# MengRao/pollnet

Measured on AMD Instinct MI355X. Metric: device-resident Gbit/s + Mframes/s, 1500 B IPv4/TCP frames, 1/2/4/8 MI355X, higher is better.
Workload: dtype u16/u32 integer (one's-complement sums)

## Files before the change

include/pollnet_amd.h:

```cpp
#ifndef POLLNET_AMD_H
#define POLLNET_AMD_H

#include <stdint.h>

#ifdef __cplusplus
extern "C" {
#endif

#define PN_ABI_VERSION 1

#define PN_RECV_BUF_SIZE 2048u
#define PN_RECV_MSS 1460u
#define PN_EMPTY_KEY (1ull << 63)
#define PN_MISS 0xFFFFFFFFu

#define PN_OK 0
#define PN_EINVAL -1
#define PN_EHIP -2
#define PN_ENOMEM -3
#define PN_ENOTABLE -4
#define PN_EFULL -5
#define PN_ENOENT -6

typedef struct pn_result {
  uint32_t conn_id;
  uint32_t seq;
  uint16_t payload_off;
  int16_t payload_len;
  uint16_t flags;
  uint16_t tcp_fold;
} pn_result;

#define PN_F_IP_OK 0x0001u
#define PN_F_TCP_OK 0x0002u
#define PN_F_HIT 0x0004u
#define PN_F_TW 0x0008u
#define PN_F_FIN 0x0010u
#define PN_F_SYN 0x0020u
#define PN_F_RST 0x0040u
#define PN_F_PSH 0x0080u
#define PN_F_ACK 0x0100u
#define PN_F_IHL_NE_5 0x0200u
#define PN_F_RFC_IP_OK 0x0400u
#define PN_F_RFC_TCP_OK 0x0800u
#define PN_F_NOT_TCP 0x1000u
#define PN_F_TRUNC 0x2000u
#define PN_F_BADOFF 0x4000u
#define PN_F_TCP_UNCHECKED 0x8000u

typedef struct pn_conn_entry {
  uint64_t key;
  uint32_t conn_id;
  uint32_t _pad;
} pn_conn_entry;

typedef struct pn_conn_table pn_conn_table;

uint64_t pn_conn_hash_key(uint32_t ip_be, uint16_t port_be);

int pn_table_create(uint32_t max_conn_cnt, uint32_t max_tw_cnt, pn_conn_table** out);
#define PN_TABLE_REFERENCE_LITERAL 1u
int pn_table_create_ex(uint32_t max_conn_cnt, uint32_t max_tw_cnt, uint32_t flags, pn_conn_table** out);
uint32_t pn_table_flags(const pn_conn_table* t);
void pn_table_destroy(pn_conn_table* t);
int pn_table_find(const pn_conn_table* t, uint64_t key, uint32_t* entry_idx, int* hit, uint32_t* conn_id);
int pn_table_add(pn_conn_table* t, uint64_t key, uint32_t conn_id);
int pn_table_del(pn_conn_table* t, uint64_t key);
int pn_table_set_conn_id(pn_conn_table* t, uint64_t key, uint32_t conn_id);
const pn_conn_entry* pn_table_entries(const pn_conn_table* t, uint32_t* n_entries, uint64_t* tbl_mask);
uint32_t pn_table_max_conn_cnt(const pn_conn_table* t);
uint32_t pn_table_size(const pn_conn_table* t);
uint32_t pn_table_repairs(const pn_conn_table* t);

typedef struct pn_ctx pn_ctx;

int pn_open(int device, pn_ctx** out);
void pn_close(pn_ctx* ctx);
const char* pn_last_error(const pn_ctx* ctx);
int pn_device_count(int* n);

int pn_set_conn_table(pn_ctx* ctx, const pn_conn_entry* entries, uint32_t n_entries, uint64_t tbl_mask,
                      uint32_t max_conn_cnt);

int pn_set_verify(pn_ctx* ctx, int verify_tcp);

int pn_classify(pn_ctx* ctx, const void* frames_dev, uint32_t slot_stride, uint32_t frame_off, uint32_t n,
                void* results_dev, void* stream);

int pn_classify_indexed(pn_ctx* ctx, const void* base, const uint64_t* offsets, uint32_t eth_mod16, uint32_t n,
                        uint32_t avail, void* results, void* stream);

#define PN_MAX_STREAM_FILTERS 64
#define PN_NO_STREAM 0xFFFFFFFFu
typedef struct pn_stream_filter {
  uint32_t src_ip;
  uint32_t dst_ip;
  uint16_t src_port;
  uint16_t dst_port;
  uint32_t _pad;
} pn_stream_filter;

int pn_match_streams(pn_ctx* ctx, const void* frames, uint32_t slot_stride, uint32_t frame_off, uint32_t n,
                     const pn_stream_filter* filters, uint32_t n_filters, uint32_t* stream_ids, void* stream);

#define PN_UDP_MAX_SUBS 4096u
#define PN_UDP_NO_SUB 0xFFFFFFFFu
typedef struct pn_udp_sub {
  uint32_t dst_ip;
  uint16_t dst_port;
  uint16_t _pad;
} pn_udp_sub;

typedef struct pn_udp_result {
  uint32_t sub_id;
  uint32_t src_ip;
  uint16_t src_port;
  uint16_t payload_off;
  uint16_t payload_len;
  uint16_t flags;
} pn_udp_result;

#define PN_UF_IP_OK 0x0001u
#define PN_UF_UDP_OK 0x0002u
#define PN_UF_MATCH 0x0004u
#define PN_UF_NOCSUM 0x0008u
#define PN_UF_FRAG 0x0010u
#define PN_UF_LEN_BAD 0x0020u
#define PN_UF_IHL_NE_5 0x0200u
#define PN_UF_NOT_UDP 0x1000u
#define PN_UF_TRUNC 0x2000u
#define PN_UF_BADOFF 0x4000u
#define PN_UF_UDP_UNCHECKED 0x8000u
#define PN_UDP_DELIVER(f) (((f) & PN_UF_MATCH) && ((f) & PN_UF_IP_OK) && \
                           ((f) & (PN_UF_UDP_OK | PN_UF_NOCSUM | PN_UF_UDP_UNCHECKED)))

int pn_udp_set_subs(pn_ctx* ctx, const pn_udp_sub* subs, uint32_t n_subs);
int pn_udp_classify(pn_ctx* ctx, const void* frames, uint32_t slot_stride, uint32_t frame_off, uint32_t n,
                    void* results, void* stream);
int pn_udp_classify_indexed(pn_ctx* ctx, const void* base, const uint64_t* offsets, uint32_t eth_mod16,
                            uint32_t n, uint32_t avail, void* results, void* stream);

#define PN_UDP_MAX_CHANNELS 4096u
typedef struct pn_udp_channel {
  uint8_t hdr[42];
  uint8_t _pad[6];
} pn_udp_channel;

#define PN_UB_EFVI 0u
#define PN_UB_PLAIN 1u
#define PN_UB_CSUM 2u

int pn_udp_set_channels(pn_ctx* ctx, const pn_udp_channel* chans, uint32_t n_chans);
int pn_udp_build(pn_ctx* ctx, const void* payloads, uint64_t payload_bytes, const uint64_t* pay_offs,
                 const uint16_t* pay_lens, const uint32_t* chan_ids, void* frames, uint32_t slot_stride,
                 uint32_t frame_off, uint32_t n, uint32_t mode, uint16_t* frame_lens, void* stream);

#define PN_UDP_GATHER_ALIGN 16u
typedef struct pn_udp_gather_total {
  uint64_t n_bytes;
  uint32_t n_msgs;
  uint32_t n_fit;
} pn_udp_gather_total;

int pn_udp_gather(pn_ctx* ctx, const void* frames, uint32_t slot_stride, uint32_t frame_off, uint32_t n,
                  const void* results, void* payloads, uint64_t payload_cap, uint64_t* pay_offs, uint16_t* pay_lens,
                  uint32_t* sub_ids, uint32_t* src_index, pn_udp_gather_total* total, void* stream);
int pn_udp_gather_indexed(pn_ctx* ctx, const void* base, const uint64_t* offsets, uint32_t eth_mod16, uint32_t n,
                          uint32_t avail, const void* results, void* payloads, uint64_t payload_cap,
                          uint64_t* pay_offs, uint16_t* pay_lens, uint32_t* sub_ids, uint32_t* src_index,
                          pn_udp_gather_total* total, void* stream);

#define PN_TX_TCP 0u
#define PN_TX_UDP_EFVI 1u
#define PN_TX_UDP 2u
int pn_tx_fill(pn_ctx* ctx, void* frames, uint32_t slot_stride, uint32_t frame_off, uint32_t n, const uint16_t* lens,
               uint32_t mode, void* stream);

#define PN_NOTIFY_MAX_FRAMES 1024u
int pn_classify_notify(pn_ctx* ctx, const void* frames, uint32_t slot_stride, uint32_t frame_off, uint32_t n,
                       void* results, void* stream, uint32_t* done_word, uint32_t token);
int pn_tx_fill_notify(pn_ctx* ctx, void* frames, uint32_t slot_stride, uint32_t frame_off, uint32_t n,
                      const uint16_t* lens, uint32_t mode, void* stream, uint32_t* done_word, uint32_t token);

typedef struct pn_service pn_service;
#define PN_SERVICE_WAVES 64u
#define PN_SERVICE_WAVES_PER_CU 12u
#define PN_SERVICE_MAX_WAVES 4096u
#define PN_SERVICE_MAX_FRAMES (1u << 20)
#define PN_SERVICE_STOP 0xFFFFFFFFu
int pn_service_open(pn_ctx* ctx, uint32_t slot_stride, uint32_t frame_off, uint32_t idle_ms, pn_service** out);
int pn_service_open_ex(pn_ctx* ctx, uint32_t slot_stride, uint32_t frame_off, uint32_t idle_ms, uint32_t large_waves,
                       pn_service** out);
int pn_service_post(pn_service* svc, const void* frames, uint32_t n, void* results, uint32_t* post_id);
#define PN_LINK_MAX_FRAMES 1024u
#define PN_LINK_MAX_CONNS 4096u
int pn_service_post_linked(pn_service* svc, const void* frames, uint32_t n, void* results, uint16_t* links,
                           uint32_t* post_id);
int pn_service_wait(pn_service* svc, uint32_t post_id);
int pn_service_close(pn_service* svc);

int pn_sync(pn_ctx* ctx);

#ifdef __cplusplus
}
#endif
#endif
```

pollnet_amd/__init__.py:

```python
from .rx import (
    LIB_PATH,
    PN_EMPTY_KEY,
    PN_MISS,
    PN_TX_TCP,
    PN_TX_UDP_EFVI,
    PN_TX_UDP,
    RESULT_DTYPE,
    ENTRY_DTYPE,
    STREAM_FILTER_DTYPE,
    PN_NO_STREAM,
    PN_MAX_STREAM_FILTERS,
    UDP_SUB_DTYPE,
    UDP_RESULT_DTYPE,
    PN_UDP_NO_SUB,
    PN_UDP_MAX_SUBS,
    UDP_CHANNEL_DTYPE,
    PN_UDP_MAX_CHANNELS,
    UDP_GATHER_TOTAL_DTYPE,
    PN_UDP_GATHER_ALIGN,
    PN_UB_EFVI,
    PN_UB_PLAIN,
    PN_UB_CSUM,
    UF,
    PN_SERVICE_WAVES,
    PN_SERVICE_WAVES_PER_CU,
    PN_SERVICE_MAX_WAVES,
    PN_SERVICE_MAX_FRAMES,
    PN_LINK_MAX_FRAMES,
    PN_LINK_MAX_CONNS,
    F,
    ConnTable,
    PollnetError,
    RxContext,
    RxService,
    conn_hash_key,
    device_count,
    gen_conn_table,
    gen_frames,
    wire_bytes,
)
```

pollnet_amd/csrc/conn_table.cpp:

```cpp
#include <algorithm>
#include <cstdint>
#include <cstring>
#include <new>
#include <utility>
#include <vector>

#include "../../include/pollnet_amd.h"

namespace {

constexpr int msb_count(uint32_t n) { return n == 0 ? 0 : msb_count(n >> 1) + 1; }

struct ConnTable {
  std::vector<pn_conn_entry> tbl;
  uint64_t mask = 0;
  uint32_t max_conn = 0, max_tw = 0, size = 0;
  uint32_t repairs = 0;
  bool literal = false;

  bool init(uint32_t mc, uint32_t mtw, bool lit) {
    literal = lit;
    max_conn = mc;
    max_tw = mtw;
    uint64_t max_tbl = 1ull << (1 + msb_count(mc + mtw));
    if (max_tbl > (1ull << 28)) return false;
    tbl.assign(max_tbl + mc + mtw, pn_conn_entry{PN_EMPTY_KEY, 0, 0});
    mask = std::min<uint64_t>(max_tbl, 128) - 1;
    size = 0;
    return true;
  }

  uint32_t find(uint64_t key) const {
    uint64_t e = key & mask;
    const uint64_t n = tbl.size();
    while (e < n && tbl[e].key < key) ++e;
    return (uint32_t)e;
  }

  void insert_sorted(uint64_t key, uint32_t conn_id) {
    uint32_t e = find(key);
    while (tbl[e].key != PN_EMPTY_KEY) {
      std::swap(tbl[e].key, key);
      std::swap(tbl[e].conn_id, conn_id);
      while (tbl[++e].key < key) {
      }
    }
    tbl[e].key = key;
    tbl[e].conn_id = conn_id;
  }

  void expand() {
    if ((uint64_t)size * 2 <= mask) return;
    std::vector<pn_conn_entry> saved;
    saved.reserve(size);
    for (const auto& x : tbl)
      if (x.key != PN_EMPTY_KEY) saved.push_back(x);
    bool broken = false;
    uint64_t end = mask + 1;
    mask = mask * 2 + 1;
    uint64_t new_end = mask + 1;
    while (tbl[end].key != PN_EMPTY_KEY) std::swap(tbl[new_end++], tbl[end++]);
    const uint64_t end_cnt = new_end - (mask + 1);
    auto rehash = [&](uint64_t e, uint64_t cnt) {
      for (; cnt; ++e) {
        if (tbl[e].key == PN_EMPTY_KEY) continue;
        uint32_t ne = find(tbl[e].key);
        if (tbl[ne].key != tbl[e].key && tbl[ne].key != PN_EMPTY_KEY) broken = true;
        std::swap(tbl[e].key, tbl[ne].key);
        tbl[ne].conn_id = tbl[e].conn_id;
        --cnt;
      }
    };
    rehash(0, size - end_cnt);
    rehash(mask + 1, end_cnt);
    if (broken && !literal) {
      ++repairs;
      for (auto& x : tbl) x = pn_conn_entry{PN_EMPTY_KEY, 0, 0};
      for (const auto& x : saved) insert_sorted(x.key, x.conn_id);
    }
  }

  int add(uint64_t key, uint32_t conn_id) {
    uint32_t e = find(key);
    if (e < tbl.size() && tbl[e].key == key) return PN_EINVAL;
    if (size >= max_conn + max_tw) return PN_EFULL;
    ++size;
    insert_sorted(key, conn_id);
    expand();
    return PN_OK;
  }

  int del(uint64_t key) {
    uint32_t e = find(key);
    if (e >= tbl.size() || tbl[e].key != key) return PN_ENOENT;
    --size;
    for (;;) {
      uint32_t next = e + 1;
      while ((tbl[next].key & mask) > e) ++next;
      if (tbl[next].key == PN_EMPTY_KEY) break;
      tbl[e] = tbl[next];
      e = next;
    }
    tbl[e].key = PN_EMPTY_KEY;
    return PN_OK;
  }
};

}

struct pn_conn_table {
  ConnTable t;
};

extern "C" {

uint64_t pn_conn_hash_key(uint32_t ip_be, uint16_t port_be) {
  uint64_t ip = __builtin_bswap32(ip_be);
  uint64_t p = __builtin_bswap16(port_be);
  return (ip << 15) | (p & 0x7fff) | ((p & 0x8000) << 32);
}

int pn_table_create(uint32_t max_conn_cnt, uint32_t max_tw_cnt, pn_conn_table** out) {
  return pn_table_create_ex(max_conn_cnt, max_tw_cnt, 0, out);
}

int pn_table_create_ex(uint32_t max_conn_cnt, uint32_t max_tw_cnt, uint32_t flags, pn_conn_table** out) {
  if (!out || max_conn_cnt == 0 || (flags & ~PN_TABLE_REFERENCE_LITERAL)) return PN_EINVAL;
  auto* t = new (std::nothrow) pn_conn_table();
  if (!t) return PN_ENOMEM;
  if (!t->t.init(max_conn_cnt, max_tw_cnt, flags & PN_TABLE_REFERENCE_LITERAL)) {
    delete t;
    return PN_EINVAL;
  }
  *out = t;
  return PN_OK;
}

void pn_table_destroy(pn_conn_table* t) { delete t; }

int pn_table_find(const pn_conn_table* t, uint64_t key, uint32_t* entry_idx, int* hit, uint32_t* conn_id) {
  if (!t) return PN_EINVAL;
  uint32_t e = t->t.find(key);
  bool h = e < t->t.tbl.size() && t->t.tbl[e].key == key;
  if (entry_idx) *entry_idx = e;
  if (hit) *hit = h;
  if (conn_id) *conn_id = h ? t->t.tbl[e].conn_id : PN_MISS;
  return PN_OK;
}

int pn_table_add(pn_conn_table* t, uint64_t key, uint32_t conn_id) {
  if (!t || key >= PN_EMPTY_KEY) return PN_EINVAL;
  return t->t.add(key, conn_id);
}

int pn_table_del(pn_conn_table* t, uint64_t key) {
  if (!t) return PN_EINVAL;
  return t->t.del(key);
}

int pn_table_set_conn_id(pn_conn_table* t, uint64_t key, uint32_t conn_id) {
  if (!t) return PN_EINVAL;
  uint32_t e = t->t.find(key);
  if (e >= t->t.tbl.size() || t->t.tbl[e].key != key) return PN_ENOENT;
  t->t.tbl[e].conn_id = conn_id;
  return PN_OK;
}

const pn_conn_entry* pn_table_entries(const pn_conn_table* t, uint32_t* n_entries, uint64_t* tbl_mask) {
  if (!t) return nullptr;
  if (n_entries) *n_entries = (uint32_t)t->t.tbl.size();
  if (tbl_mask) *tbl_mask = t->t.mask;
  return t->t.tbl.data();
}

uint32_t pn_table_max_conn_cnt(const pn_conn_table* t) { return t ? t->t.max_conn : 0; }
uint32_t pn_table_size(const pn_conn_table* t) { return t ? t->t.size : 0; }
uint32_t pn_table_repairs(const pn_conn_table* t) { return t ? t->t.repairs : 0; }
uint32_t pn_table_flags(const pn_conn_table* t) { return t && t->t.literal ? PN_TABLE_REFERENCE_LITERAL : 0u; }

}
```

pollnet_amd/csrc/pn_internal.hpp:

```cpp
#pragma once

#include <hip/hip_runtime.h>

#include <cstdint>
#include <string>
#include <vector>

#include "../../include/pollnet_amd.h"

struct pn_fence {
  hipStream_t s = nullptr;
  hipEvent_t ev = nullptr;
  uint8_t state = 0;
};

struct pn_ctx {
  int device = 0;
  pn_conn_entry* tbl_buf[2] = {nullptr, nullptr};
  uint32_t tbl_cap[2] = {0, 0};
  int cur = 0;
  pn_conn_entry* tbl_dev = nullptr;
  uint32_t n_entries = 0;
  uint64_t mask = 0;
  uint32_t max_conn = 0;
  bool verify_tcp = true;
  std::vector<hipStream_t> streams;
  std::vector<hipEvent_t> retired;
  size_t n_retired = 0;
  hipStream_t copy_stream = nullptr;
  void* tx_patch = nullptr;
  uint32_t tx_patch_n = 0;
  pn_fence tx;
  void* sig_count = nullptr;
  pn_fence sig[2];
  std::vector<pn_service*> services;
  uint64_t* udp_tbl = nullptr;
  uint32_t udp_cap = 0;
  uint32_t udp_mask = 0;
  uint32_t udp_n = 0;
  uint32_t* ub_tbl = nullptr;
  uint32_t ub_cap = 0;
  uint32_t ub_n = 0;
  void* ug_scratch = nullptr;
  uint32_t ug_scratch_n = 0;
  pn_fence ug;
  std::string err;
};

namespace pn_internal {

inline thread_local std::string g_err;

inline int set_err(pn_ctx* ctx, int code, const std::string& msg) {
  if (ctx) ctx->err = msg;
  g_err = msg;
  return code;
}

int svc_release_table(pn_ctx* ctx, int buf);

inline int hip_err(pn_ctx* ctx, hipError_t e, const char* what) {
  return set_err(ctx, PN_EHIP, std::string(what) + ": " + hipGetErrorString(e));
}

inline void note_stream(pn_ctx* ctx, hipStream_t s) {
  if (!ctx->streams.empty() && ctx->streams.back() == s) return;
  for (size_t i = 0; i < ctx->streams.size(); ++i)
    if (ctx->streams[i] == s) {
      std::swap(ctx->streams[i], ctx->streams.back());
      return;
    }
  ctx->streams.push_back(s);
}

inline int ensure_event(pn_ctx* ctx, hipEvent_t* ev) {
  if (*ev) return PN_OK;
  hipError_t e = hipEventCreateWithFlags(ev, hipEventDisableTiming);
  if (e != hipSuccess) return hip_err(ctx, e, "hipEventCreate");
  return PN_OK;
}

inline int fence_host_wait(pn_ctx* ctx, pn_fence& f) {
  hipError_t e = hipSuccess;
  if (f.state == 1) e = hipStreamSynchronize(f.s);
  else if (f.state == 2) e = hipEventSynchronize(f.ev);
  if (e != hipSuccess) return hip_err(ctx, e, "waiting for the last user of ctx scratch");
  f.state = 0;
  return PN_OK;
}

inline int fence_use(pn_ctx* ctx, pn_fence& f, hipStream_t s) {
  hipError_t e = hipSuccess;
  if (f.state == 1 && f.s != s) {
    int rc = ensure_event(ctx, &f.ev);
    if (rc) return rc;
    e = hipEventRecord(f.ev, f.s);
    if (e == hipSuccess) e = hipStreamWaitEvent(s, f.ev, 0);
  } else if (f.state == 2) {
    e = hipStreamWaitEvent(s, f.ev, 0);
  }
  if (e != hipSuccess) return hip_err(ctx, e, "ordering after the previous user of ctx scratch");
  f.s = s;
  f.state = 1;
  return PN_OK;
}

inline int fence_detach(pn_ctx* ctx, pn_fence& f) {
  if (f.state != 1) return PN_OK;
  int rc = ensure_event(ctx, &f.ev);
  if (rc) return rc;
  hipError_t e = hipEventRecord(f.ev, f.s);
  if (e != hipSuccess) return hip_err(ctx, e, "hipEventRecord(ctx scratch fence)");
  f.state = 2;
  f.s = nullptr;
  return PN_OK;
}

inline int wait_retired(pn_ctx* ctx) {
  for (size_t i = 0; i < ctx->n_retired; ++i) {
    hipError_t e = hipEventSynchronize(ctx->retired[i]);
    if (e != hipSuccess) return hip_err(ctx, e, "hipEventSynchronize(previous table readers)");
  }
  ctx->n_retired = 0;
  return PN_OK;
}

inline int retire_streams(pn_ctx* ctx) {
  for (size_t i = 0; i < ctx->streams.size(); ++i) {
    if (ctx->retired.size() <= i) ctx->retired.push_back(nullptr);
    int rc = ensure_event(ctx, &ctx->retired[i]);
    if (rc) return rc;
    hipError_t e = hipEventRecord(ctx->retired[i], ctx->streams[i]);
    if (e != hipSuccess) return hip_err(ctx, e, "hipEventRecord(table readers)");
  }
  ctx->n_retired = ctx->streams.size();
  ctx->streams.clear();
  for (pn_fence* f : {&ctx->sig[0], &ctx->sig[1], &ctx->tx, &ctx->ug}) {
    int rc = fence_detach(ctx, *f);
    if (rc) return rc;
  }
  return PN_OK;
}

inline int notify_counter(pn_ctx* ctx, int kind, hipStream_t s, uint32_t** out) {
  hipError_t e;
  if (!ctx->sig_count) {
    e = hipMalloc(&ctx->sig_count, 128);
    if (e == hipSuccess) e = hipMemsetAsync(ctx->sig_count, 0, 128, s);
    if (e != hipSuccess) return hip_err(ctx, e, "hipMalloc(notify counters)");
    for (pn_fence& f : ctx->sig) {
      f.s = s;
      f.state = 1;
    }
    note_stream(ctx, s);
  }
  int rc = fence_use(ctx, ctx->sig[kind], s);
  if (rc) return rc;
  *out = (uint32_t*)ctx->sig_count + 16 * kind;
  return PN_OK;
}

}
```

pollnet_amd/csrc/rx_kernel.hip:

```cpp
#include "rx_classify.hpp"

namespace {
using pn_internal::g_err;
using pn_internal::hip_err;
using pn_internal::set_err;

int strided_args(pn_ctx* ctx, const char* fn, const void* frames_dev, uint32_t slot_stride, uint32_t frame_off,
                 uint32_t n, void* results_dev, KArgs& a) {
  if (!ctx) return set_err(nullptr, PN_EINVAL, std::string(fn) + ": ctx is NULL");
  if (!ctx->tbl_dev) return set_err(ctx, PN_ENOTABLE, std::string(fn) + ": no conn table (call pn_set_conn_table)");
  if (!frames_dev || !results_dev) return set_err(ctx, PN_EINVAL, std::string(fn) + ": NULL buffer");
  if (((uintptr_t)frames_dev & 15) || ((uintptr_t)results_dev & 15))
    return set_err(ctx, PN_EINVAL, std::string(fn) + ": frames/results must be 16-byte aligned");
  if ((slot_stride & 15) || slot_stride > 65536 || (frame_off & 1) || slot_stride < frame_off + 96)
    return set_err(ctx, PN_EINVAL, std::string(fn) + ": slot_stride/frame_off violate the layout contract");
  strided_kargs(a, frames_dev, results_dev, ctx->tbl_dev, ctx->mask, ctx->n_entries, ctx->max_conn, n, slot_stride, frame_off);
  return PN_OK;
}

template <bool SIG>
void launch_strided(const pn_ctx* ctx, const KArgs& a, uint32_t frame_off, hipStream_t s) {
  for_mis(frame_off, [&](auto mis) {
    if (ctx->verify_tcp) launch<mis(), SIG, false>(a, s);
    else launch<mis(), SIG, true>(a, s);
  });
}

template <int A>
void launch_indexed(const KArgs& a, uint32_t eth_mod16, hipStream_t s) {
  for_mis(eth_mod16, [&](auto mis) { launch_one<mis(), 1, A, kLoadAux, kStoreAux, 1, kIdxWin, kXcdOrder>(a, s); });
}

}

extern "C" {

int pn_device_count(int* n) {
  if (!n) return PN_EINVAL;
  hipError_t e = hipGetDeviceCount(n);
  if (e != hipSuccess) {
    *n = 0;
    return hip_err(nullptr, e, "hipGetDeviceCount");
  }
  return PN_OK;
}


int pn_open(int device, pn_ctx** out) {
  if (!out) return set_err(nullptr, PN_EINVAL, "pn_open: out is NULL");
  int n = 0;
  hipError_t e = hipGetDeviceCount(&n);
  if (e != hipSuccess) return hip_err(nullptr, e, "hipGetDeviceCount");
  if (device < 0 || device >= n) return set_err(nullptr, PN_EINVAL, "pn_open: no such device");
  pn_ctx* c = new pn_ctx();
  c->device = device;
  *out = c;
  return PN_OK;
}

void pn_close(pn_ctx* ctx) {
  if (!ctx) return;
  (void)hipSetDevice(ctx->device);
  if (ctx->tbl_buf[0] || ctx->tbl_buf[1] || ctx->tx_patch || ctx->sig_count || ctx->udp_tbl || ctx->ub_tbl ||
      ctx->ug_scratch)
    (void)hipDeviceSynchronize();
  for (pn_conn_entry* b : ctx->tbl_buf)
    if (b) (void)hipFree(b);
  if (ctx->udp_tbl) (void)hipFree(ctx->udp_tbl);
  if (ctx->ub_tbl) (void)hipFree(ctx->ub_tbl);
  if (ctx->tx_patch) (void)hipFree(ctx->tx_patch);
  if (ctx->ug_scratch) (void)hipFree(ctx->ug_scratch);
  if (ctx->sig_count) (void)hipFree(ctx->sig_count);
  for (hipEvent_t ev : ctx->retired)
    if (ev) (void)hipEventDestroy(ev);
  for (pn_fence* f : {&ctx->sig[0], &ctx->sig[1], &ctx->tx, &ctx->ug})
    if (f->ev) (void)hipEventDestroy(f->ev);
  if (ctx->copy_stream) (void)hipStreamDestroy(ctx->copy_stream);
  delete ctx;
}

const char* pn_last_error(const pn_ctx* ctx) { return ctx ? ctx->err.c_str() : g_err.c_str(); }

int pn_set_conn_table(pn_ctx* ctx, const pn_conn_entry* entries, uint32_t n_entries, uint64_t tbl_mask,
                      uint32_t max_conn_cnt) {
  if (!ctx || !entries || n_entries == 0) return set_err(ctx, PN_EINVAL, "pn_set_conn_table: bad arguments");
  if (tbl_mask >= n_entries || (tbl_mask & (tbl_mask + 1)) != 0)
    return set_err(ctx, PN_EINVAL, "pn_set_conn_table: tbl_mask must be 2^k-1 < n_entries");
  hipError_t e = hipSetDevice(ctx->device);
  if (e != hipSuccess) return hip_err(ctx, e, "hipSetDevice");
  const int nxt = ctx->tbl_dev ? ctx->cur ^ 1 : ctx->cur;
  int rc = pn_internal::svc_release_table(ctx, nxt);
  if (rc) return rc;
  rc = pn_internal::wait_retired(ctx);
  if (rc) return rc;
  if (n_entries > ctx->tbl_cap[nxt]) {
    if (ctx->tbl_buf[nxt]) (void)hipFree(ctx->tbl_buf[nxt]);
    ctx->tbl_buf[nxt] = nullptr;
    ctx->tbl_cap[nxt] = 0;
    e = hipMalloc(&ctx->tbl_buf[nxt], (size_t)n_entries * sizeof(pn_conn_entry));
    if (e != hipSuccess) return hip_err(ctx, e, "hipMalloc(conn table)");
    ctx->tbl_cap[nxt] = n_entries;
  }
  if (!ctx->copy_stream) {
    e = hipStreamCreateWithFlags(&ctx->copy_stream, hipStreamNonBlocking);
    if (e != hipSuccess) return hip_err(ctx, e, "hipStreamCreate(table uploads)");
  }
  e = hipMemcpyAsync(ctx->tbl_buf[nxt], entries, (size_t)n_entries * sizeof(pn_conn_entry), hipMemcpyHostToDevice,
                     ctx->copy_stream);
  if (e == hipSuccess) e = hipStreamSynchronize(ctx->copy_stream);
  if (e != hipSuccess) return hip_err(ctx, e, "hipMemcpyAsync(conn table)");
  rc = pn_internal::retire_streams(ctx);
  if (rc) return rc;
  ctx->cur = nxt;
  ctx->tbl_dev = ctx->tbl_buf[nxt];
  ctx->n_entries = n_entries;
  ctx->mask = tbl_mask;
  ctx->max_conn = max_conn_cnt;
  return PN_OK;
}


int pn_classify(pn_ctx* ctx, const void* frames_dev, uint32_t slot_stride, uint32_t frame_off, uint32_t n,
                void* results_dev, void* stream) {
  if (ctx && n == 0 && ctx->tbl_dev) return PN_OK;
  KArgs a;
  int rc = strided_args(ctx, "pn_classify", frames_dev, slot_stride, frame_off, n, results_dev, a);
  if (rc) return rc;
  if (n == 0) return PN_OK;
  hipStream_t s = (hipStream_t)stream;
  hipError_t e = hipSetDevice(ctx->device);
  if (e != hipSuccess) return hip_err(ctx, e, "hipSetDevice");
  launch_strided<false>(ctx, a, frame_off, s);
  e = hipGetLastError();
  if (e != hipSuccess) return hip_err(ctx, e, "rx_classify launch");
  pn_internal::note_stream(ctx, s);
  return PN_OK;
}

int pn_classify_notify(pn_ctx* ctx, const void* frames, uint32_t slot_stride, uint32_t frame_off, uint32_t n,
                       void* results, void* stream, uint32_t* done_word, uint32_t token) {
  KArgs a;
  int rc = strided_args(ctx, "pn_classify_notify", frames, slot_stride, frame_off, n, results, a);
  if (rc) return rc;
  if (n == 0 || n > PN_NOTIFY_MAX_FRAMES || !done_word || ((uintptr_t)done_word & 3))
    return set_err(ctx, PN_EINVAL, "pn_classify_notify: n must be in [1, PN_NOTIFY_MAX_FRAMES], done_word 4-byte aligned");
  hipStream_t s = (hipStream_t)stream;
  hipError_t e = hipSetDevice(ctx->device);
  if (e != hipSuccess) return hip_err(ctx, e, "hipSetDevice");
  rc = pn_internal::notify_counter(ctx, 0, s, &a.sig_count);
  if (rc) return rc;
  a.sig_flag = done_word;
  a.sig_token = token;
  launch_strided<true>(ctx, a, frame_off, s);
  e = hipGetLastError();
  if (e != hipSuccess) return hip_err(ctx, e, "rx_classify (notify) launch");
  pn_internal::note_stream(ctx, s);
  return PN_OK;
}


int pn_classify_indexed(pn_ctx* ctx, const void* base, const uint64_t* offsets, uint32_t eth_mod16, uint32_t n,
                        uint32_t avail, void* results_dev, void* stream) {
  if (!ctx) return set_err(nullptr, PN_EINVAL, "pn_classify_indexed: ctx is NULL");
  if (!ctx->tbl_dev) return set_err(ctx, PN_ENOTABLE, "pn_classify_indexed: no conn table (call pn_set_conn_table)");
  if (n == 0) return PN_OK;
  if (!base || !offsets || !results_dev) return set_err(ctx, PN_EINVAL, "pn_classify_indexed: NULL buffer");
  if (((uintptr_t)base & 15) || ((uintptr_t)results_dev & 15) || ((uintptr_t)offsets & 7))
    return set_err(ctx, PN_EINVAL, "pn_classify_indexed: base/results must be 16-byte, offsets 8-byte aligned");
  if (eth_mod16 > 15 || (eth_mod16 & 1) || avail < 96 || avail > 65536)
    return set_err(ctx, PN_EINVAL, "pn_classify_indexed: eth_mod16 must be even < 16, avail in [96, 65536]");
  KArgs a;
  a.frames = (const uint8_t*)base;
  a.out = (pn_result*)results_dev;
  a.tbl = ctx->tbl_dev;
  a.mask = ctx->mask;
  a.n_entries = ctx->n_entries;
  a.max_conn = ctx->max_conn;
  a.n = n;
  a.stride = 0;
  a.ipa_off = 0;
  a.avail = avail;
  a.offs = offsets;
  a.fpw = frames_per_wave(n);
  hipStream_t s = (hipStream_t)stream;
  hipError_t e = hipSetDevice(ctx->device);
  if (e != hipSuccess) return hip_err(ctx, e, "hipSetDevice");
  if (ctx->verify_tcp) launch_indexed<kProdAbl>(a, eth_mod16, s);
  else launch_indexed<kProdAbl | kHeaderOnly>(a, eth_mod16, s);
  e = hipGetLastError();
  if (e != hipSuccess) return hip_err(ctx, e, "rx_classify (indexed) launch");
  pn_internal::note_stream(ctx, s);
  return PN_OK;
}

int pn_set_verify(pn_ctx* ctx, int verify_tcp) {
  if (!ctx) return set_err(nullptr, PN_EINVAL, "pn_set_verify: ctx is NULL");
  ctx->verify_tcp = verify_tcp != 0;
  return PN_OK;
}

int pn_sync(pn_ctx* ctx) {
  if (!ctx) return set_err(nullptr, PN_EINVAL, "pn_sync: ctx is NULL");
  hipError_t e = hipSetDevice(ctx->device);
  if (e != hipSuccess) return hip_err(ctx, e, "hipSetDevice");
  for (hipStream_t s : ctx->streams) {
    e = hipStreamSynchronize(s);
    if (e != hipSuccess) return hip_err(ctx, e, "hipStreamSynchronize");
  }
  ctx->streams.clear();
  int rc = pn_internal::wait_retired(ctx);
  if (rc) return rc;
  for (pn_fence* f : {&ctx->sig[0], &ctx->sig[1], &ctx->tx, &ctx->ug}) f->state = 0;
  return PN_OK;
}

}
```

pollnet_amd/rx.py:

```python
from __future__ import annotations

import ctypes
import os
from dataclasses import dataclass

import numpy as np

LIB_PATH = os.path.join(os.path.dirname(os.path.abspath(__file__)), "libpollnet_amd.so")

PN_EMPTY_KEY = 1 << 63
PN_MISS = 0xFFFFFFFF
PN_RECV_BUF_SIZE = 2048
PN_TX_TCP = 0
PN_TX_UDP_EFVI = 1
PN_TX_UDP = 2
PN_NOTIFY_MAX_FRAMES = 1024


class F:

    IP_OK = 0x0001
    TCP_OK = 0x0002
    HIT = 0x0004
    TW = 0x0008
    FIN = 0x0010
    SYN = 0x0020
    RST = 0x0040
    PSH = 0x0080
    ACK = 0x0100
    IHL_NE_5 = 0x0200
    RFC_IP_OK = 0x0400
    RFC_TCP_OK = 0x0800
    NOT_TCP = 0x1000
    TRUNC = 0x2000
    BADOFF = 0x4000
    TCP_UNCHECKED = 0x8000


RESULT_DTYPE = np.dtype(
    [("conn_id", "<u4"), ("seq", "<u4"), ("payload_off", "<u2"), ("payload_len", "<i2"), ("flags", "<u2"), ("tcp_fold", "<u2")]
)
ENTRY_DTYPE = np.dtype([("key", "<u8"), ("conn_id", "<u4"), ("_pad", "<u4")])
STREAM_FILTER_DTYPE = np.dtype([("src_ip", "<u4"), ("dst_ip", "<u4"), ("src_port", "<u2"), ("dst_port", "<u2"),
                                ("_pad", "<u4")])
PN_NO_STREAM = 0xFFFFFFFF
PN_MAX_STREAM_FILTERS = 64
assert RESULT_DTYPE.itemsize == 16 and ENTRY_DTYPE.itemsize == 16 and STREAM_FILTER_DTYPE.itemsize == 16

UDP_SUB_DTYPE = np.dtype([("dst_ip", "<u4"), ("dst_port", "<u2"), ("_pad", "<u2")])
UDP_RESULT_DTYPE = np.dtype([("sub_id", "<u4"), ("src_ip", "<u4"), ("src_port", "<u2"), ("payload_off", "<u2"),
                             ("payload_len", "<u2"), ("flags", "<u2")])
PN_UDP_NO_SUB = 0xFFFFFFFF
PN_UDP_MAX_SUBS = 4096
assert UDP_SUB_DTYPE.itemsize == 8 and UDP_RESULT_DTYPE.itemsize == 16
UDP_CHANNEL_DTYPE = np.dtype([("hdr", "u1", (42,)), ("_pad", "u1", (6,))])
PN_UDP_MAX_CHANNELS = 4096
PN_UB_EFVI = 0
PN_UB_PLAIN = 1
PN_UB_CSUM = 2
assert UDP_CHANNEL_DTYPE.itemsize == 48
UDP_GATHER_TOTAL_DTYPE = np.dtype([("n_bytes", "<u8"), ("n_msgs", "<u4"), ("n_fit", "<u4")])
PN_UDP_GATHER_ALIGN = 16
assert UDP_GATHER_TOTAL_DTYPE.itemsize == 16


class UF:

    IP_OK = 0x0001
    UDP_OK = 0x0002
    MATCH = 0x0004
    NOCSUM = 0x0008
    FRAG = 0x0010
    LEN_BAD = 0x0020
    IHL_NE_5 = 0x0200
    NOT_UDP = 0x1000
    TRUNC = 0x2000
    BADOFF = 0x4000
    UDP_UNCHECKED = 0x8000

    @staticmethod
    def deliver(flags):
        f = np.asarray(flags)
        return ((f & UF.MATCH) != 0) & ((f & UF.IP_OK) != 0) & ((f & (UF.UDP_OK | UF.NOCSUM | UF.UDP_UNCHECKED)) != 0)


class PollnetError(RuntimeError):
    pass


def _load():
    try:
        import torch
    except ImportError:
        pass
    if not os.path.exists(LIB_PATH):
        raise ImportError(
            f"{LIB_PATH} not built: run `make` (or __graft_entry__.build()); there is no CPU fallback for the RX path"
        )
    return ctypes.CDLL(LIB_PATH)


_lib = _load()
_c = ctypes
_vp, _u32, _u64, _i32, _u16 = _c.c_void_p, _c.c_uint32, _c.c_uint64, _c.c_int, _c.c_uint16


class _GenParams(_c.Structure):
    _fields_ = [("cfg", _u32), ("n_flows", _u32), ("n_tw_flows", _u32), ("max_conn_cnt", _u32), ("seed", _u64)]


def _sig(name, res, *args):
    fn = getattr(_lib, name)
    fn.restype = res
    fn.argtypes = list(args)
    return fn


_pn_conn_hash_key = _sig("pn_conn_hash_key", _u64, _u32, _u16)
_pn_table_create = _sig("pn_table_create", _i32, _u32, _u32, _c.POINTER(_vp))
_pn_table_create_ex = _sig("pn_table_create_ex", _i32, _u32, _u32, _u32, _c.POINTER(_vp))
_pn_table_flags = _sig("pn_table_flags", _u32, _vp)
_pn_table_destroy = _sig("pn_table_destroy", None, _vp)
_pn_table_find = _sig("pn_table_find", _i32, _vp, _u64, _c.POINTER(_u32), _c.POINTER(_i32), _c.POINTER(_u32))
_pn_table_add = _sig("pn_table_add", _i32, _vp, _u64, _u32)
_pn_table_del = _sig("pn_table_del", _i32, _vp, _u64)
_pn_table_set_conn_id = _sig("pn_table_set_conn_id", _i32, _vp, _u64, _u32)
_pn_table_entries = _sig("pn_table_entries", _vp, _vp, _c.POINTER(_u32), _c.POINTER(_u64))
_pn_table_max_conn_cnt = _sig("pn_table_max_conn_cnt", _u32, _vp)
_pn_table_size = _sig("pn_table_size", _u32, _vp)
_pn_table_repairs = _sig("pn_table_repairs", _u32, _vp)
_pn_open = _sig("pn_open", _i32, _i32, _c.POINTER(_vp))
_pn_close = _sig("pn_close", None, _vp)
_pn_last_error = _sig("pn_last_error", _c.c_char_p, _vp)
_pn_device_count = _sig("pn_device_count", _i32, _c.POINTER(_i32))
_pn_set_conn_table = _sig("pn_set_conn_table", _i32, _vp, _vp, _u32, _u64, _u32)
_pn_classify = _sig("pn_classify", _i32, _vp, _vp, _u32, _u32, _u32, _vp, _vp)
_pn_classify_indexed = _sig("pn_classify_indexed", _i32, _vp, _vp, _vp, _u32, _u32, _u32, _vp, _vp)
_pn_tx_fill = _sig("pn_tx_fill", _i32, _vp, _vp, _u32, _u32, _u32, _vp, _u32, _vp)
_pn_classify_notify = _sig("pn_classify_notify", _i32, _vp, _vp, _u32, _u32, _u32, _vp, _vp, _vp, _u32)
_pn_tx_fill_notify = _sig("pn_tx_fill_notify", _i32, _vp, _vp, _u32, _u32, _u32, _vp, _u32, _vp, _vp, _u32)
_pn_sync = _sig("pn_sync", _i32, _vp)
_pn_set_verify = _sig("pn_set_verify", _i32, _vp, _i32)
_pn_match_streams = _sig("pn_match_streams", _i32, _vp, _vp, _u32, _u32, _u32, _vp, _u32, _vp, _vp)
_pn_udp_set_subs = _sig("pn_udp_set_subs", _i32, _vp, _vp, _u32)
_pn_udp_classify = _sig("pn_udp_classify", _i32, _vp, _vp, _u32, _u32, _u32, _vp, _vp)
_pn_udp_classify_indexed = _sig("pn_udp_classify_indexed", _i32, _vp, _vp, _vp, _u32, _u32, _u32, _vp, _vp)
_pn_udp_set_channels = _sig("pn_udp_set_channels", _i32, _vp, _vp, _u32)
_pn_udp_build = _sig("pn_udp_build", _i32, _vp, _vp, _u64, _vp, _vp, _vp, _vp, _u32, _u32, _u32, _u32, _vp, _vp)
_pn_udp_gather = _sig("pn_udp_gather", _i32, _vp, _vp, _u32, _u32, _u32, _vp, _vp, _u64, _vp, _vp, _vp, _vp, _vp, _vp)
_pn_udp_gather_indexed = _sig("pn_udp_gather_indexed", _i32, _vp, _vp, _vp, _u32, _u32, _u32, _vp, _vp, _u64, _vp, _vp,
                              _vp, _vp, _vp, _vp)
_pn_service_open = _sig("pn_service_open", _i32, _vp, _u32, _u32, _u32, _c.POINTER(_vp))
_pn_service_open_ex = _sig("pn_service_open_ex", _i32, _vp, _u32, _u32, _u32, _u32, _c.POINTER(_vp))
_pn_service_post = _sig("pn_service_post", _i32, _vp, _vp, _u32, _vp, _vp)
_pn_service_post_linked = _sig("pn_service_post_linked", _i32, _vp, _vp, _u32, _vp, _vp, _vp)
_pn_service_wait = _sig("pn_service_wait", _i32, _vp, _u32)
_pn_service_close = _sig("pn_service_close", _i32, _vp)
PN_SERVICE_WAVES = 64
PN_SERVICE_WAVES_PER_CU = 12
PN_SERVICE_MAX_WAVES = 4096
PN_LINK_MAX_FRAMES = 1024
PN_LINK_MAX_CONNS = 4096
PN_SERVICE_MAX_FRAMES = 1 << 20

GEN_LIB_PATH = os.path.join(os.path.dirname(os.path.abspath(__file__)), "libpollnet_amd_gen.so")
_gen = {}


def _gen_fn(name, res, *args):
    if not _gen:
        if not os.path.exists(GEN_LIB_PATH):
            raise ImportError(f"{GEN_LIB_PATH} not built: run `make`")
        _gen["lib"] = ctypes.CDLL(GEN_LIB_PATH)
    fn = getattr(_gen["lib"], name)
    fn.restype = res
    fn.argtypes = list(args)
    return fn


def _check(rc, ctx=None, what=""):
    if rc != 0:
        msg = _pn_last_error(ctx).decode(errors="replace")
        raise PollnetError(f"{what} failed ({rc}): {msg}")


def conn_hash_key(ip_be: int, port_be: int) -> int:
    return int(_pn_conn_hash_key(ip_be & 0xFFFFFFFF, port_be & 0xFFFF))


def device_count() -> int:
    n = _i32(0)
    _pn_device_count(_c.byref(n))
    return n.value


PN_TABLE_REFERENCE_LITERAL = 1


class ConnTable:

    def __init__(self, max_conn_cnt: int, max_tw_cnt: int, reference_literal: bool = False):
        h = _vp()
        flags = PN_TABLE_REFERENCE_LITERAL if reference_literal else 0
        _check(_pn_table_create_ex(max_conn_cnt, max_tw_cnt, flags, _c.byref(h)), None, "pn_table_create_ex")
        self._h = h
        self.reference_literal = bool(_pn_table_flags(h) & PN_TABLE_REFERENCE_LITERAL)

    def __del__(self):
        if getattr(self, "_h", None):
            _pn_table_destroy(self._h)
            self._h = None

    @property
    def handle(self):
        return self._h

    def find(self, key: int):
        idx, hit, cid = _u32(), _i32(), _u32()
        _check(_pn_table_find(self._h, key, _c.byref(idx), _c.byref(hit), _c.byref(cid)), None, "pn_table_find")
        return idx.value, bool(hit.value), cid.value

    def add(self, key: int, conn_id: int):
        _check(_pn_table_add(self._h, key, conn_id), None, "pn_table_add")

    def delete(self, key: int):
        _check(_pn_table_del(self._h, key), None, "pn_table_del")

    def set_conn_id(self, key: int, conn_id: int):
        _check(_pn_table_set_conn_id(self._h, key, conn_id), None, "pn_table_set_conn_id")

    @property
    def max_conn_cnt(self) -> int:
        return int(_pn_table_max_conn_cnt(self._h))

    @property
    def size(self) -> int:
        return int(_pn_table_size(self._h))

    @property
    def repairs(self) -> int:
        return int(_pn_table_repairs(self._h))

    def snapshot(self):
        n, mask = _u32(), _u64()
        p = _pn_table_entries(self._h, _c.byref(n), _c.byref(mask))
        buf = (_c.c_uint8 * (n.value * 16)).from_address(p)
        return np.frombuffer(bytes(buf), dtype=ENTRY_DTYPE).copy(), int(mask.value)

    @property
    def mask(self) -> int:
        return self.snapshot()[1]


def _ptr(x):
    if x is None:
        return None
    if isinstance(x, int):
        return x
    if hasattr(x, "data_ptr"):
        return x.data_ptr()
    if isinstance(x, np.ndarray):
        return x.ctypes.data
    raise TypeError(f"cannot take the address of {type(x)}")


def _hold(ctx, stream):
    h = _stream_handle(stream)
    if h is not None and not isinstance(stream, int) and h not in ctx._held:
        ctx._held[h] = stream
    return h


def _stream_handle(stream):
    if stream is None:
        return None
    if isinstance(stream, int):
        return stream
    return stream.cuda_stream


class RxContext:

    def __init__(self, device: int = 0):
        h = _vp()
        _check(_pn_open(device, _c.byref(h)), None, "pn_open")
        self._h = h
        self.device = device
        self.max_conn_cnt = 0
        self._held = {}

    def close(self):
        if getattr(self, "_h", None):
            _pn_close(self._h)
            self._h = None

    __del__ = close

    def set_conn_table(self, table: ConnTable):
        entries, mask = table.snapshot()
        self.set_conn_entries(entries, mask, table.max_conn_cnt)

    def set_conn_entries(self, entries: np.ndarray, mask: int, max_conn_cnt: int):
        entries = np.ascontiguousarray(entries, dtype=ENTRY_DTYPE)
        _check(
            _pn_set_conn_table(self._h, entries.ctypes.data, len(entries), mask, max_conn_cnt), self._h, "pn_set_conn_table"
        )
        self.max_conn_cnt = max_conn_cnt
        self._held.clear()

    def set_verify(self, verify_tcp: bool):
        _check(_pn_set_verify(self._h, 1 if verify_tcp else 0), self._h, "pn_set_verify")

    def classify(self, frames_dev, slot_stride: int, frame_off: int, n: int, results_dev, stream=None):
        _check(
            _pn_classify(self._h, _ptr(frames_dev), slot_stride, frame_off, n, _ptr(results_dev), _hold(self, stream)),
            self._h,
            "pn_classify",
        )

    def classify_notify(self, frames, slot_stride: int, frame_off: int, n: int, results, done_word, token: int,
                        stream=None):
        _check(_pn_classify_notify(self._h, _ptr(frames), slot_stride, frame_off, n, _ptr(results),
                                   _hold(self, stream), _ptr(done_word), token), self._h, "pn_classify_notify")

    def tx_fill_notify(self, frames, slot_stride: int, frame_off: int, n: int, done_word, token: int, lens=None,
                       mode: int = PN_TX_TCP, stream=None):
        _check(_pn_tx_fill_notify(self._h, _ptr(frames), slot_stride, frame_off, n, _ptr(lens), mode,
                                  _hold(self, stream), _ptr(done_word), token), self._h, "pn_tx_fill_notify")

    def classify_indexed(self, base, offsets, eth_mod16: int, n: int, avail: int, results, stream=None):
        _check(
            _pn_classify_indexed(self._h, _ptr(base), _ptr(offsets), eth_mod16, n, avail, _ptr(results),
                                 _hold(self, stream)),
            self._h,
            "pn_classify_indexed",
        )

    def tx_fill(self, frames_dev, slot_stride: int, frame_off: int, n: int, lens=None, mode: int = PN_TX_TCP,
                stream=None):
        _check(_pn_tx_fill(self._h, _ptr(frames_dev), slot_stride, frame_off, n, _ptr(lens), mode,
                           _hold(self, stream)), self._h, "pn_tx_fill")

    def match_streams(self, frames, slot_stride: int, frame_off: int, n: int, filters: np.ndarray, stream_ids,
                      stream=None):
        flt = np.ascontiguousarray(filters, dtype=STREAM_FILTER_DTYPE)
        _check(_pn_match_streams(self._h, _ptr(frames), slot_stride, frame_off, n, flt.ctypes.data, len(flt),
                                 _ptr(stream_ids), _hold(self, stream)), self._h, "pn_match_streams")

    def udp_set_subs(self, subs: np.ndarray):
        s = np.ascontiguousarray(subs, dtype=UDP_SUB_DTYPE)
        _check(_pn_udp_set_subs(self._h, s.ctypes.data, len(s)), self._h, "pn_udp_set_subs")
        self._held.clear()

    def udp_classify(self, frames, slot_stride: int, frame_off: int, n: int, results, stream=None):
        _check(_pn_udp_classify(self._h, _ptr(frames), slot_stride, frame_off, n, _ptr(results), _hold(self, stream)),
               self._h, "pn_udp_classify")

    def udp_classify_indexed(self, base, offsets, eth_mod16: int, n: int, avail: int, results, stream=None):
        _check(
            _pn_udp_classify_indexed(self._h, _ptr(base), _ptr(offsets), eth_mod16, n, avail, _ptr(results),
                                     _hold(self, stream)),
            self._h,
            "pn_udp_classify_indexed",
        )

    def udp_set_channels(self, chans: np.ndarray):
        c = np.ascontiguousarray(chans, dtype=UDP_CHANNEL_DTYPE)
        _check(_pn_udp_set_channels(self._h, c.ctypes.data, len(c)), self._h, "pn_udp_set_channels")
        self._held.clear()

    def udp_build(self, payloads, payload_bytes: int, pay_offs, pay_lens, chan_ids, frames, slot_stride: int,
                  frame_off: int, n: int, mode: int, frame_lens, stream=None):
        _check(
            _pn_udp_build(self._h, _ptr(payloads), payload_bytes, _ptr(pay_offs), _ptr(pay_lens),
                          None if chan_ids is None else _ptr(chan_ids), _ptr(frames), slot_stride, frame_off, n, mode,
                          _ptr(frame_lens), _hold(self, stream)),
            self._h,
            "pn_udp_build",
        )

    def udp_gather(self, frames, slot_stride: int, frame_off: int, n: int, results, payloads, payload_cap: int,
                   pay_offs, pay_lens, sub_ids, src_index, total, stream=None):
        _check(
            _pn_udp_gather(self._h, _ptr(frames), slot_stride, frame_off, n, _ptr(results), _ptr(payloads), payload_cap,
                           _ptr(pay_offs), _ptr(pay_lens), _ptr(sub_ids), None if src_index is None else _ptr(src_index),
                           _ptr(total), _hold(self, stream)),
            self._h,
            "pn_udp_gather",
        )

    def udp_gather_indexed(self, base, offsets, eth_mod16: int, n: int, avail: int, results, payloads,
                           payload_cap: int, pay_offs, pay_lens, sub_ids, src_index, total, stream=None):
        _check(
            _pn_udp_gather_indexed(self._h, _ptr(base), _ptr(offsets), eth_mod16, n, avail, _ptr(results),
                                   _ptr(payloads), payload_cap, _ptr(pay_offs), _ptr(pay_lens), _ptr(sub_ids),
                                   None if src_index is None else _ptr(src_index), _ptr(total), _hold(self, stream)),
            self._h,
            "pn_udp_gather_indexed",
        )

    def sync(self):
        _check(_pn_sync(self._h), self._h, "pn_sync")
        self._held.clear()


@dataclass
class GenParams:
    cfg: int
    n_flows: int = 1024
    n_tw_flows: int = 0
    max_conn_cnt: int = 1024
    seed: int = 0

    @staticmethod
    def for_config(cfg: int) -> "GenParams":
        seeds = {2: 0x5EED0002, 3: 0x5EED0003, 4: 0x5EED0004, 5: 0x5EED0005}
        if cfg == 2:
            return GenParams(2, 1, 0, 1024, seeds[2])
        if cfg == 4:
            return GenParams(4, 1024, 0, 1024, seeds[4])
        return GenParams(cfg, 1024, 32, 1024, seeds[cfg])

    def _c(self):
        return _GenParams(self.cfg, self.n_flows, self.n_tw_flows, self.max_conn_cnt, self.seed)


def gen_frames(params: GenParams, n: int, slot_stride: int = PN_RECV_BUF_SIZE, frame_off: int = 2, first_index: int = 0,
               threads: int = 0, out: np.ndarray | None = None) -> np.ndarray:
    if out is None:
        out = np.empty((n, slot_stride), dtype=np.uint8)
    assert out.dtype == np.uint8 and out.flags.c_contiguous and out.size >= n * slot_stride
    threads = threads or min(16, os.cpu_count() or 1)
    p = params._c()
    gen = _gen_fn("pn_gen_frames", _i32, _c.POINTER(_GenParams), _u64, _u32, _vp, _u32, _u32, _i32)
    _check(gen(_c.byref(p), first_index, n, out.ctypes.data, slot_stride, frame_off, threads), None, "pn_gen_frames")
    return out


def gen_conn_table(params: GenParams, max_tw_cnt: int | None = None) -> ConnTable:
    t = ConnTable(params.max_conn_cnt, params.max_conn_cnt if max_tw_cnt is None else max_tw_cnt)
    p = params._c()
    _check(_gen_fn("pn_gen_conn_table", _i32, _c.POINTER(_GenParams), _vp)(_c.byref(p), t.handle), None,
           "pn_gen_conn_table")
    return t


def wire_bytes(slots: np.ndarray, slot_stride: int, frame_off: int, n: int) -> int:
    return int(_gen_fn("pn_wire_bytes", _u64, _vp, _u32, _u32, _u32)(slots.ctypes.data, slot_stride, frame_off, n))


class RxService:

    def __init__(self, ctx: RxContext, slot_stride: int, frame_off: int, idle_ms: int = 200, large_waves: int = 0):
        h = _vp()
        _check(_pn_service_open_ex(ctx._h, slot_stride, frame_off, idle_ms, large_waves, _c.byref(h)), ctx._h,
               "pn_service_open")
        self._h, self._ctx = h, ctx
        self._inflight = {}
        self._last = None

    def post(self, frames, n: int, results, links=None) -> int:
        pid = _u32(0)
        if links is None:
            rc = _pn_service_post(self._h, _ptr(frames), n, _ptr(results), _c.byref(pid))
        else:
            rc = _pn_service_post_linked(self._h, _ptr(frames), n, _ptr(results), _ptr(links), _c.byref(pid))
        _check(rc, self._ctx._h, "pn_service_post")
        self._inflight[pid.value] = (frames, results, links)
        self._last = pid.value
        return pid.value

    def wait(self, post_id: int = 0):
        _check(_pn_service_wait(self._h, post_id), self._ctx._h, "pn_service_wait")
        last = post_id or self._last
        if last is None:
            return
        for k in [k for k in self._inflight if ((last - k) & 0xFFFFFFFF) < 0x80000000]:
            del self._inflight[k]

    def classify(self, frames, n: int, results, links=None):
        self.post(frames, n, results, links)
        self.wait()

    def close(self):
        if getattr(self, "_h", None):
            h, self._h = self._h, None
            try:
                _check(_pn_service_close(h), self._ctx._h, "pn_service_close")
            finally:
                self._inflight.clear()

    def __del__(self):
        try:
            self.close()
        except Exception:
            pass
```

Before: 53790.

## Widen device connection hash table to shorten GPU probe chains

```diff
diff --git a/include/pollnet_amd.h b/include/pollnet_amd.h
--- a/include/pollnet_amd.h
+++ b/include/pollnet_amd.h
@@ -72,6 +72,10 @@
 uint32_t pn_table_size(const pn_conn_table* t);
 uint32_t pn_table_repairs(const pn_conn_table* t);
 
+#define PN_TABLE_WIDE_MAX_ENTRIES (1u << 17)
+int pn_table_widen(const pn_conn_entry* entries, uint32_t n_entries, uint64_t tbl_mask, uint32_t spread,
+                   pn_conn_entry* out, uint32_t out_cap, uint32_t* out_n, uint64_t* out_mask);
+
 typedef struct pn_ctx pn_ctx;
 
 int pn_open(int device, pn_ctx** out);
@@ -81,6 +85,9 @@
 
 int pn_set_conn_table(pn_ctx* ctx, const pn_conn_entry* entries, uint32_t n_entries, uint64_t tbl_mask,
                       uint32_t max_conn_cnt);
+
+#define PN_TABLE_SPREAD_DEFAULT 32u
+int pn_set_table_spread(pn_ctx* ctx, uint32_t factor);
 
 int pn_set_verify(pn_ctx* ctx, int verify_tcp);
 
diff --git a/pollnet_amd/__init__.py b/pollnet_amd/__init__.py
--- a/pollnet_amd/__init__.py
+++ b/pollnet_amd/__init__.py
@@ -38,4 +38,7 @@
     gen_conn_table,
     gen_frames,
     wire_bytes,
+    widen_table,
+    PN_TABLE_SPREAD_DEFAULT,
+    PN_TABLE_WIDE_MAX_ENTRIES,
 )
diff --git a/pollnet_amd/csrc/conn_table.cpp b/pollnet_amd/csrc/conn_table.cpp
--- a/pollnet_amd/csrc/conn_table.cpp
+++ b/pollnet_amd/csrc/conn_table.cpp
@@ -10,6 +10,24 @@
 namespace {
 
 constexpr int msb_count(uint32_t n) { return n == 0 ? 0 : msb_count(n >> 1) + 1; }
+
+uint64_t walk(const pn_conn_entry* tbl, uint64_t n, uint64_t mask, uint64_t key) {
+  uint64_t e = key & mask;
+  while (e < n && tbl[e].key < key) ++e;
+  return e;
+}
+
+void insert_ordered(pn_conn_entry* tbl, uint64_t n, uint64_t mask, uint64_t key, uint32_t conn_id) {
+  uint64_t e = walk(tbl, n, mask, key);
+  while (tbl[e].key != PN_EMPTY_KEY) {
+    std::swap(tbl[e].key, key);
+    std::swap(tbl[e].conn_id, conn_id);
+    while (tbl[++e].key < key) {
+    }
+  }
+  tbl[e].key = key;
+  tbl[e].conn_id = conn_id;
+}
 
 struct ConnTable {
   std::vector<pn_conn_entry> tbl;
@@ -30,24 +48,9 @@
     return true;
   }
 
-  uint32_t find(uint64_t key) const {
-    uint64_t e = key & mask;
-    const uint64_t n = tbl.size();
-    while (e < n && tbl[e].key < key) ++e;
-    return (uint32_t)e;
-  }
-
-  void insert_sorted(uint64_t key, uint32_t conn_id) {
-    uint32_t e = find(key);
-    while (tbl[e].key != PN_EMPTY_KEY) {
-      std::swap(tbl[e].key, key);
-      std::swap(tbl[e].conn_id, conn_id);
-      while (tbl[++e].key < key) {
-      }
-    }
-    tbl[e].key = key;
-    tbl[e].conn_id = conn_id;
-  }
+  uint32_t find(uint64_t key) const { return (uint32_t)walk(tbl.data(), tbl.size(), mask, key); }
+
+  void insert_sorted(uint64_t key, uint32_t conn_id) { insert_ordered(tbl.data(), tbl.size(), mask, key, conn_id); }
 
   void expand() {
     if ((uint64_t)size * 2 <= mask) return;
@@ -178,4 +181,33 @@
 uint32_t pn_table_repairs(const pn_conn_table* t) { return t ? t->t.repairs : 0; }
 uint32_t pn_table_flags(const pn_conn_table* t) { return t && t->t.literal ? PN_TABLE_REFERENCE_LITERAL : 0u; }
 
-}
+int pn_table_widen(const pn_conn_entry* entries, uint32_t n_entries, uint64_t tbl_mask, uint32_t spread,
+                   pn_conn_entry* out, uint32_t out_cap, uint32_t* out_n, uint64_t* out_mask) {
+  if (!entries || n_entries == 0 || !out_n || !out_mask || tbl_mask >= n_entries || (tbl_mask & (tbl_mask + 1)) != 0)
+    return PN_EINVAL;
+  uint64_t cap = tbl_mask + 1;
+  uint64_t live = 0;
+  if (spread > 1 && cap < PN_TABLE_WIDE_MAX_ENTRIES) {
+    for (uint32_t i = 0; i < n_entries; ++i) live += entries[i].key < PN_EMPTY_KEY;
+    while (cap < PN_TABLE_WIDE_MAX_ENTRIES && cap < spread * live) cap <<= 1;
+    if (cap + live > UINT32_MAX) cap = tbl_mask + 1;
+  }
+  const bool wide = cap != tbl_mask + 1;
+  const uint64_t n = wide ? cap + live : n_entries;
+  *out_n = (uint32_t)n;
+  *out_mask = cap - 1;
+  if (!out) return PN_OK;
+  if (out_cap < n) return PN_EINVAL;
+  if (!wide) {
+    std::memcpy(out, entries, n * sizeof(pn_conn_entry));
+    return PN_OK;
+  }
+  std::fill(out, out + n, pn_conn_entry{PN_EMPTY_KEY, 0, 0});
+  for (uint32_t i = 0; i < n_entries; ++i) {
+    const uint64_t k = entries[i].key;
+    if (k < PN_EMPTY_KEY && walk(entries, n_entries, tbl_mask, k) == i) insert_ordered(out, n, cap - 1, k, entries[i].conn_id);
+  }
+  return PN_OK;
+}
+
+}
diff --git a/pollnet_amd/csrc/pn_internal.hpp b/pollnet_amd/csrc/pn_internal.hpp
--- a/pollnet_amd/csrc/pn_internal.hpp
+++ b/pollnet_amd/csrc/pn_internal.hpp
@@ -23,6 +23,10 @@
   uint32_t n_entries = 0;
   uint64_t mask = 0;
   uint32_t max_conn = 0;
+  uint32_t src_n_entries = 0;
+  uint64_t src_mask = 0;
+  uint32_t spread = PN_TABLE_SPREAD_DEFAULT;
+  std::vector<pn_conn_entry> wide;
   bool verify_tcp = true;
   std::vector<hipStream_t> streams;
   std::vector<hipEvent_t> retired;
diff --git a/pollnet_amd/csrc/rx_kernel.hip b/pollnet_amd/csrc/rx_kernel.hip
--- a/pollnet_amd/csrc/rx_kernel.hip
+++ b/pollnet_amd/csrc/rx_kernel.hip
@@ -86,6 +86,20 @@
   if (!ctx || !entries || n_entries == 0) return set_err(ctx, PN_EINVAL, "pn_set_conn_table: bad arguments");
   if (tbl_mask >= n_entries || (tbl_mask & (tbl_mask + 1)) != 0)
     return set_err(ctx, PN_EINVAL, "pn_set_conn_table: tbl_mask must be 2^k-1 < n_entries");
+  const uint32_t src_n_entries = n_entries;
+  const uint64_t src_mask = tbl_mask;
+  uint32_t wide_n = 0;
+  uint64_t wide_mask = 0;
+  if (pn_table_widen(entries, n_entries, tbl_mask, ctx->spread, nullptr, 0, &wide_n, &wide_mask) != PN_OK)
+    return set_err(ctx, PN_EINVAL, "pn_set_conn_table: bad arguments");
+  if (wide_mask != tbl_mask) {
+    if (ctx->wide.size() < wide_n) ctx->wide.resize(wide_n);
+    if (pn_table_widen(entries, n_entries, tbl_mask, ctx->spread, ctx->wide.data(), wide_n, &wide_n, &wide_mask) != PN_OK)
+      return set_err(ctx, PN_EINVAL, "pn_set_conn_table: widening the table failed");
+    entries = ctx->wide.data();
+    n_entries = wide_n;
+    tbl_mask = wide_mask;
+  }
   hipError_t e = hipSetDevice(ctx->device);
   if (e != hipSuccess) return hip_err(ctx, e, "hipSetDevice");
   const int nxt = ctx->tbl_dev ? ctx->cur ^ 1 : ctx->cur;
@@ -116,6 +130,14 @@
   ctx->n_entries = n_entries;
   ctx->mask = tbl_mask;
   ctx->max_conn = max_conn_cnt;
+  ctx->src_n_entries = src_n_entries;
+  ctx->src_mask = src_mask;
+  return PN_OK;
+}
+
+int pn_set_table_spread(pn_ctx* ctx, uint32_t factor) {
+  if (!ctx) return set_err(nullptr, PN_EINVAL, "pn_set_table_spread: ctx is NULL");
+  ctx->spread = factor;
   return PN_OK;
 }
 
diff --git a/pollnet_amd/rx.py b/pollnet_amd/rx.py
--- a/pollnet_amd/rx.py
+++ b/pollnet_amd/rx.py
@@ -129,6 +129,10 @@
 _pn_table_max_conn_cnt = _sig("pn_table_max_conn_cnt", _u32, _vp)
 _pn_table_size = _sig("pn_table_size", _u32, _vp)
 _pn_table_repairs = _sig("pn_table_repairs", _u32, _vp)
+_pn_table_widen = _sig("pn_table_widen", _i32, _vp, _u32, _u64, _u32, _vp, _u32, _c.POINTER(_u32), _c.POINTER(_u64))
+_pn_set_table_spread = _sig("pn_set_table_spread", _i32, _vp, _u32)
+PN_TABLE_SPREAD_DEFAULT = 32
+PN_TABLE_WIDE_MAX_ENTRIES = 1 << 17
 _pn_open = _sig("pn_open", _i32, _i32, _c.POINTER(_vp))
 _pn_close = _sig("pn_close", None, _vp)
 _pn_last_error = _sig("pn_last_error", _c.c_char_p, _vp)
@@ -252,6 +256,17 @@
         return self.snapshot()[1]
 
 
+def widen_table(entries: np.ndarray, mask: int, spread: int = PN_TABLE_SPREAD_DEFAULT):
+    entries = np.ascontiguousarray(entries, dtype=ENTRY_DTYPE)
+    n, m = _u32(), _u64()
+    _check(_pn_table_widen(entries.ctypes.data, len(entries), mask, spread, None, 0, _c.byref(n), _c.byref(m)), None,
+           "pn_table_widen")
+    out = np.empty(n.value, ENTRY_DTYPE)
+    _check(_pn_table_widen(entries.ctypes.data, len(entries), mask, spread, out.ctypes.data, len(out), _c.byref(n),
+                           _c.byref(m)), None, "pn_table_widen")
+    return out, int(m.value)
+
+
 def _ptr(x):
     if x is None:
         return None
@@ -308,6 +323,9 @@
         self.max_conn_cnt = max_conn_cnt
         self._held.clear()
 
+    def set_table_spread(self, factor: int):
+        _check(_pn_set_table_spread(self._h, factor), self._h, "pn_set_table_spread")
+
     def set_verify(self, verify_tcp: bool):
         _check(_pn_set_verify(self._h, 1 if verify_tcp else 0), self._h, "pn_set_verify")
 
```

Result: no change. 53780 (-0.0%).
